# MatchaChoco010/toy-cpu-pathtracing

Hardware: NVIDIA B200
Metric: Mrays/s (higher is better)
Workload: dtype f32

## Files before the change

toy_cpu_pathtracing_b200/csrc/dcommon.cuh:

```cuda
#pragma once
#include <cuda_runtime.h>
#include <stdint.h>

#include "../../include/tcpt_flat.h"

namespace tcpt {

#define TCPT_PI 3.14159265358979323846f
#define TCPT_FLT_MAX 3.402823466e+38f
#define TCPT_INF __int_as_float(0x7f800000)

__device__ __forceinline__ float3 f3(float x, float y, float z) { return make_float3(x, y, z); }
__device__ __forceinline__ float3 operator+(float3 a, float3 b) { return f3(a.x + b.x, a.y + b.y, a.z + b.z); }
__device__ __forceinline__ float3 operator-(float3 a, float3 b) { return f3(a.x - b.x, a.y - b.y, a.z - b.z); }
__device__ __forceinline__ float3 operator-(float3 a) { return f3(-a.x, -a.y, -a.z); }
__device__ __forceinline__ float3 operator*(float3 a, float s) { return f3(a.x * s, a.y * s, a.z * s); }
__device__ __forceinline__ float3 operator*(float s, float3 a) { return f3(s * a.x, s * a.y, s * a.z); }
__device__ __forceinline__ float3 operator/(float3 a, float s) { return f3(a.x / s, a.y / s, a.z / s); }
__device__ __forceinline__ float dot(float3 a, float3 b) { return (a.x * b.x) + (a.y * b.y) + (a.z * b.z); }
__device__ __forceinline__ float3 cross(float3 a, float3 b) { return f3(a.y * b.z - b.y * a.z, a.z * b.x - b.z * a.x, a.x * b.y - b.x * a.y); }
__device__ __forceinline__ float length_squared(float3 a) { return dot(a, a); }
__device__ __forceinline__ float length(float3 a) { return sqrtf(dot(a, a)); }
__device__ __forceinline__ float3 normalize(float3 a) { return a * (1.0f / length(a)); }
__device__ __forceinline__ float comp(float3 a, int i) { return i == 0 ? a.x : (i == 1 ? a.y : a.z); }
// ... 11 lines not shown
    return f3((m[0] * v.x + m[3] * v.y) + m[6] * v.z, (m[1] * v.x + m[4] * v.y) + m[7] * v.z, (m[2] * v.x + m[5] * v.y) + m[8] * v.z);
}
__device__ __forceinline__ float3 xf_normal_by_inverse(const float* __restrict__ inv, float3 n) {
    float3 r = f3((inv[0] * n.x + inv[1] * n.y) + inv[2] * n.z, (inv[3] * n.x + inv[4] * n.y) + inv[5] * n.z, (inv[6] * n.x + inv[7] * n.y) + inv[8] * n.z);
    return normalize(r);
}

struct M3 { float3 c0, c1, c2; };
__device__ __forceinline__ M3 m3_inverse(const M3& s) {
    const float m00 = s.c0.x, m01 = s.c0.y, m02 = s.c0.z, m10 = s.c1.x, m11 = s.c1.y, m12 = s.c1.z, m20 = s.c2.x, m21 = s.c2.y, m22 = s.c2.z;
    M3 r;
    r.c0 = f3(m11 * m22 - m12 * m21, -(m01 * m22 - m02 * m21), m01 * m12 - m02 * m11);
    r.c1 = f3(-(m10 * m22 - m12 * m20), m00 * m22 - m02 * m20, -(m00 * m12 - m02 * m10));
    r.c2 = f3(m10 * m21 - m11 * m20, -(m00 * m21 - m01 * m20), m00 * m11 - m01 * m10);
    const float det = (m00 * r.c0.x + m01 * r.c1.x) + m02 * r.c2.x;
    const float rcp = 1.0f / det;
    r.c0 = r.c0 * rcp; r.c1 = r.c1 * rcp; r.c2 = r.c2 * rcp;
    return r;
}
__device__ __forceinline__ float3 m3_vector(const M3& m, float3 v) { return (m.c0 * v.x + m.c1 * v.y) + m.c2 * v.z; }
__device__ __forceinline__ float3 m3_normal_by_inverse(const M3& inv, float3 n) {
    return normalize(f3((inv.c0.x * n.x + inv.c0.y * n.y) + inv.c0.z * n.z, (inv.c1.x * n.x + inv.c1.y * n.y) + inv.c1.z * n.z,
                        (inv.c2.x * n.x + inv.c2.y * n.y) + inv.c2.z * n.z));
}

struct S4 { float v[4]; };
__device__ __forceinline__ S4 s4(float c) { S4 r; r.v[0] = r.v[1] = r.v[2] = r.v[3] = c; return r; }
__device__ __forceinline__ S4 s4(float4 a) { S4 r; r.v[0] = a.x; r.v[1] = a.y; r.v[2] = a.z; r.v[3] = a.w; return r; }
__device__ __forceinline__ float4 to_f4(const S4& a) { return make_float4(a.v[0], a.v[1], a.v[2], a.v[3]); }
#define S4_BINOP(op)                                                                                                   \
    __device__ __forceinline__ S4 operator op(const S4& a, const S4& b) { S4 r; _Pragma("unroll") for (int i = 0; i < 4; ++i) r.v[i] = a.v[i] op b.v[i]; return r; }
S4_BINOP(+) S4_BINOP(-) S4_BINOP(*)
__device__ __forceinline__ S4 operator*(const S4& a, float s) { S4 r; _Pragma("unroll") for (int i = 0; i < 4; ++i) r.v[i] = a.v[i] * s; return r; }
__device__ __forceinline__ S4 operator*(float s, const S4& a) { S4 r; _Pragma("unroll") for (int i = 0; i < 4; ++i) r.v[i] = s * a.v[i]; return r; }
__device__ __forceinline__ S4 operator/(const S4& a, float s) { S4 r; _Pragma("unroll") for (int i = 0; i < 4; ++i) r.v[i] = s == 0.0f ? 0.0f : a.v[i] / s; return r; }
__device__ __forceinline__ S4 operator/(const S4& a, const S4& b) { S4 r; _Pragma("unroll") for (int i = 0; i < 4; ++i) r.v[i] = b.v[i] == 0.0f ? 0.0f : a.v[i] / b.v[i]; return r; }
__device__ __forceinline__ float s4_max(const S4& a) { return rmax(rmax(rmax(rmax(-TCPT_INF, a.v[0]), a.v[1]), a.v[2]), a.v[3]); }
__device__ __forceinline__ float s4_avg(const S4& a) { return ((((0.0f + a.v[0]) + a.v[1]) + a.v[2]) + a.v[3]) / 4.0f; }
__device__ __forceinline__ bool s4_is_constant(const S4& a) { return a.v[1] == a.v[0] && a.v[2] == a.v[0] && a.v[3] == a.v[0]; }
__device__ __forceinline__ S4 s4_sqrt(const S4& a) { S4 r; _Pragma("unroll") for (int i = 0; i < 4; ++i) r.v[i] = sqrtf(a.v[i]); return r; }
__device__ __forceinline__ S4 s4_clamp(const S4& a, float lo, float hi) { S4 r; _Pragma("unroll") for (int i = 0; i < 4; ++i) r.v[i] = clampf(a.v[i], lo, hi); return r; }

struct DTexture { const uint8_t* data; uint32_t w, h, channels, pad; };
struct DEnv {
    const float* data; const float* marginal; const float* conditional;
    const uint32_t* marginal_guide; const uint32_t* conditional_guide; uint32_t guide_h, guide_w;
    float intensity, total_weight; uint32_t w, h; tcpt_flat_spectrum integrated; int32_t primitive;
    const float4* nee_table;
};
struct DScene {
    const float4* nodes;
    const int2* tlas_items;
    const float4* tri_verts;
    const float* positions; const float* normals; const float* uvs; const uint32_t* indices; const float* tangents;
    const tcpt_flat_geometry* geometries;
    const tcpt_flat_primitive* primitives; uint32_t n_primitives;
    const tcpt_flat_material* materials;
    const uint8_t* prim_mat_type;
    const DTexture* textures;
    const float* area_list; const float* area_table;
    int32_t light_list[TCPT_MAX_LIGHTS]; uint32_t n_lights;
    uint32_t one_light_always_on;
    const DEnv* envs; uint32_t n_envs;
    const float4* cmf;
    const float* z_nodes; const float* rgb2spec;
    float half_lin; int32_t half_zi;
    const float* presets;
    float xyz_to_rgb[9];
};

struct DCamera { float3 s, u, nf; float scale, aspect; };

struct DRender {
    uint32_t width, height, spp, seed, max_depth;
    int32_t integrator, sampler;
    float exposure;
    uint32_t log2_spp, n_base4_digits;
    uint32_t n_pix, pix_begin, s_begin, s_count, row_offset, row_stride;
    const uint32_t* pix_list;
    uint64_t n_pix_magic, width_magic;
    const uint32_t* sobol_prefix; uint32_t prefix_dims, prefix_stride;
    uint32_t pass_info;
    const unsigned long long* sobol_hash;
};
#define TCPT_SOBOL_HASH_N 512

typedef uint2 OrderEntry;

struct DState {
    float4* thr; float4* con; float4* fprev; float4* misc;
    float4* ppos;
    float4* rgb;
    float4* ext_o[2]; float4* ext_d[2];
    float4* hit0; uint2* hit1;
    float4* sh_o; float4* sh_d; float4* sh_c;
    OrderEntry* order; uint32_t capacity;
    uint32_t* counters;
    unsigned long long* stats;
};

enum : uint32_t { FLAG_SPEC_PREV = 1u, FLAG_LAMBDA_TERMINATED = 2u, FLAG_SAMPLED_PREV = 4u };

__constant__ uint32_t c_sobol_dim1[52];
__constant__ const uint32_t* c_sobol_dim1_bytes;

__device__ __forceinline__ uint32_t div_magic(uint32_t n, uint64_t magic) { return magic ? (uint32_t)__umul64hi((uint64_t)n, magic) : n; }
struct SobolFrame {
    const uint32_t* prefix;
    uint32_t prefix_stride, tables;
    uint32_t cfg;
    uint32_t seed;
    const unsigned long long* hash_table;
};
struct DSampler {
    uint32_t morton, dim, key, pix;

    __device__ __forceinline__ static uint32_t part1by1(uint32_t x) {
        x &= 0x0000ffffu;
        x = (x ^ (x << 8)) & 0x00ff00ffu;
        x = (x ^ (x << 4)) & 0x0f0f0f0fu;
        x = (x ^ (x << 2)) & 0x33333333u;
        x = (x ^ (x << 1)) & 0x55555555u;
        return x;
    }
    __device__ __forceinline__ static uint64_t mix_bits(uint64_t v) {
        v ^= v >> 31; v *= 0x7fb5d329728ea185ull; v ^= v >> 27; v *= 0x81dadef4bc2dd44dull; v ^= v >> 33;
        return v;
    }
    __device__ __forceinline__ static uint64_t hash(uint32_t dimension, uint32_t seed) {
        const uint64_t M = 0xc6a4a7935bd1e995ull;
        uint64_t h = 8ull * M;
        uint64_t k = (uint64_t)dimension | ((uint64_t)seed << 32);
        k *= M; k ^= k >> 47; k *= M;
        h ^= k; h *= M;
        h ^= h >> 47; h *= M; h ^= h >> 47;
        return h;
    }
    __device__ __forceinline__ static uint64_t hash_of(uint32_t k, const SobolFrame& f) {
        if (f.hash_table != nullptr && k < (uint32_t)TCPT_SOBOL_HASH_N) return __ldg(f.hash_table + k);
        return hash(k, f.seed);
    }
    __device__ __forceinline__ static uint32_t owen(uint32_t v, uint32_t seed) {
        v = __brev(v);
        v ^= v * 0x3d20adeau; v += seed; v *= (seed >> 16) | 1u; v ^= v * 0x05526c56u; v ^= v * 0x53a22864u;
        return __brev(v);
    }
    __device__ __forceinline__ static uint32_t pcg_hash2(uint32_t key, uint32_t ctr) {
        uint32_t x = key * 747796405u + ctr * 2891336453u + 0x9e3779b9u;
        x ^= x >> 16; x *= 0x7feb352du; x ^= x >> 15; x *= 0x846ca68bu; x ^= x >> 16;
        uint32_t w = ((x >> ((x >> 28u) + 4u)) ^ x) * 277803737u;
        return (w >> 22u) ^ w;
    }
    __device__ __forceinline__ static float unit_float(uint32_t x) { return (float)(x >> 8) * 5.9604644775390625e-8f; }
    __device__ __forceinline__ static float to_unit(uint32_t v) { return fminf((float)v * 2.3283064365386963e-10f, 0.99999994f); }

    __device__ __forceinline__ static uint32_t morton_of(uint32_t px, uint32_t py, uint32_t sample_index, uint32_t log2_spp) {
        return (((part1by1(py) << 1) | part1by1(px)) << log2_spp) | sample_index;
    }
    __device__ __forceinline__ void start(const DRender& R, uint32_t px, uint32_t py, uint32_t sample_index) {
        dim = 0;
        morton = morton_of(px, py, sample_index, R.log2_spp);
        key = (px * 0x9e3779b9u) ^ (py * 0x85ebca6bu) ^ (sample_index * 0xc2b2ae35u) ^ R.seed;
        pix = py * R.width + px;
    }
    __device__ __forceinline__ static SobolFrame frame_of(const DRender& R) {
        SobolFrame f;
// ... 344 lines not shown
```

toy_cpu_pathtracing_b200/csrc/kernels.cuh:

```cuda
#pragma once
#include "dshade.cuh"
#include "dtraverse.cuh"

#define TCPT_N_BUCKETS 9
#ifndef TCPT_SHADE_MIN_BLOCKS_LAMBERT
#define TCPT_SHADE_MIN_BLOCKS_LAMBERT 4
#endif
#ifndef TCPT_TRACE_MIN_BLOCKS
#define TCPT_TRACE_MIN_BLOCKS 8
#endif
#define TCPT_BUCKET_STRIDE 10

namespace tcpt {

struct PathList { const uint32_t* xy; const uint32_t* sample; };

__device__ __forceinline__ uint32_t owned_pixel(const DRender& R, uint32_t p_local) {
    return R.pix_list ? __ldg(R.pix_list + R.pix_begin + p_local) : R.pix_begin + p_local;
}

__device__ __forceinline__ void path_coords(const DRender& R, const PathList& L, uint32_t slot, uint32_t* px, uint32_t* py, uint32_t* si) {
    if (L.xy) { *px = __ldg(L.xy + 2 * (size_t)slot); *py = __ldg(L.xy + 2 * (size_t)slot + 1); *si = __ldg(L.sample + slot); return; }
    const uint32_t s_local = div_magic(slot, R.n_pix_magic), p_local = slot - s_local * R.n_pix;
    const uint32_t k = owned_pixel(R, p_local);
// ... 166 lines not shown
        const uint32_t b = bucket_of(sc, h.prim, killed);
        const uint32_t peers = __match_any_sync(__activemask(), b);
        const uint32_t lane = threadIdx.x & 31u;
        const int leader = __ffs(peers) - 1;
        uint32_t base = 0;
        if ((int)lane == leader) base = atomicAdd(&bcount[b], (uint32_t)__popc(peers));
        return CommitToken{base, peers, b, i, __float_as_uint(dw) & 0x7fffffffu};
    }
    __device__ __forceinline__ void end(const CommitToken& t) const {
        const uint32_t lane = threadIdx.x & 31u, peers = t.b, b = t.c, i = t.d;
        const uint32_t base = __shfl_sync(peers, t.a, __ffs(peers) - 1);
        st.order[(size_t)b * st.capacity + base + (uint32_t)__popc(peers & ((1u << lane) - 1u))] = make_uint2(i, t.e);
    }
};
struct CommitShadow {
    const DScene& sc; const DRender& R; const DState& st;
    __device__ __forceinline__ CommitToken begin(uint32_t i, const DHit& h) const {
        const uint32_t tag = __float_as_uint(st.sh_d[i].w);
        return CommitToken{tag, i, h.prim < 0 ? 1u : 0u, 0u, 0u};
    }
    __device__ __forceinline__ void end(const CommitToken& t) const {
        const uint32_t tag = t.a, i = t.b;
        const uint32_t slot = tag & 0x7fffffffu;
        const bool visible = t.c != 0u, last = (tag & 0x80000000u) != 0;
        if (!visible && !last) return;
        S4 con = s4(st.con[slot]);
        if (visible) {
            con = con + s4(st.sh_c[i]);
            st.con[slot] = to_f4(con);
        }
        if (last) {
            const float4 misc = st.misc[slot];
            const DWavelengths wl = wavelengths_uniform(misc.y, (__float_as_uint(misc.w) & FLAG_LAMBDA_TERMINATED) != 0);
            const float3 rgb = sensor_rgb(sc, wl.lambda[0], wl.terminated, con, R.exposure);
            st.rgb[slot] = make_float4(rgb.x, rgb.y, rgb.z, 0.0f);
        }
    }
};

template <bool COUNT>
__global__ void __launch_bounds__(128, 6) k_trace_closest(const __grid_constant__ DScene sc, const float4* __restrict__ q_o, const float4* __restrict__ q_d,
                                                        float4* __restrict__ hit0, uint2* __restrict__ hit1, const __grid_constant__ DState st, int cur) {
    const uint32_t n = st.counters[cur];
    uint32_t* bcount = st.counters + 4 + TCPT_BUCKET_STRIDE * cur;
    if (blockIdx.x == 0 && threadIdx.x == 0) {
        st.counters[cur ^ 1] = 0; st.counters[2] = 0; st.counters[25] = 0;
        for (int b = 0; b < TCPT_N_BUCKETS; ++b) st.counters[4 + TCPT_BUCKET_STRIDE * (cur ^ 1) + b] = 0;
        atomicAdd(&st.stats[0], (unsigned long long)n);
    }
    uint32_t nb = 0, nt = 0;
    __shared__ TraceShared ts;
    trace_queue<false, COUNT>(sc, ts, q_o, q_d, n, &st.counters[24], &nb, &nt, CommitClosest{sc, st, q_d, hit0, hit1, bcount});
    if (COUNT) { atomicAdd(&st.stats[2], (unsigned long long)nb); atomicAdd(&st.stats[3], (unsigned long long)nt); }
}

template <bool COUNT>
__global__ void __launch_bounds__(128, 6) k_trace_shadow(const __grid_constant__ DScene sc, const __grid_constant__ DRender R, const __grid_constant__ DState st) {
    const uint32_t n = st.counters[2];
    if (blockIdx.x == 0 && threadIdx.x == 0) atomicAdd(&st.stats[1], (unsigned long long)n);
    uint32_t nb = 0, nt = 0;
    __shared__ TraceShared ts;
    trace_queue<true, COUNT>(sc, ts, st.sh_o, st.sh_d, n, &st.counters[25], &nb, &nt, CommitShadow{sc, R, st});
    if (COUNT) { atomicAdd(&st.stats[2], (unsigned long long)nb); atomicAdd(&st.stats[3], (unsigned long long)nt); }
}

template <bool COUNT>
__global__ void __launch_bounds__(128, TCPT_TRACE_MIN_BLOCKS) k_trace_fused(const __grid_constant__ DScene sc, const __grid_constant__ DRender R, const __grid_constant__ DState st, int cur, int sh, uint32_t refill_lanes, uint32_t max_chunk) {
    const uint32_t n_sh = st.counters[sh], n = st.counters[cur];
    uint32_t* bcount = st.counters + 4 + TCPT_BUCKET_STRIDE * cur;
    if (blockIdx.x == 0 && threadIdx.x == 0) {
        st.counters[cur ^ 1] = 0; st.counters[sh ^ 1] = 0;
        for (int b = 0; b < TCPT_N_BUCKETS; ++b) st.counters[4 + TCPT_BUCKET_STRIDE * (cur ^ 1) + b] = 0;
        atomicAdd(&st.stats[0], (unsigned long long)n);
        atomicAdd(&st.stats[1], (unsigned long long)n_sh);
    }
    uint32_t nb = 0, nt = 0;
    __shared__ TraceShared ts;
    if (n_sh) trace_queue<true, COUNT>(sc, ts, st.sh_o, st.sh_d, n_sh, &st.counters[25], &nb, &nt, CommitShadow{sc, R, st}, refill_lanes, max_chunk);
    float4* __restrict__ hit0 = st.hit0; uint2* __restrict__ hit1 = st.hit1;
    if (n) trace_queue<false, COUNT>(sc, ts, st.ext_o[cur], st.ext_d[cur], n, &st.counters[24], &nb, &nt, CommitClosest{sc, st, st.ext_d[cur], hit0, hit1, bcount}, refill_lanes, max_chunk);
    if (COUNT) { atomicAdd(&st.stats[2], (unsigned long long)nb); atomicAdd(&st.stats[3], (unsigned long long)nt); }
}

struct ShadeOut {
    bool push_ext, push_sh;
    float4 eo, ed, so, sd, sc;
};

template <int B> struct BucketInfo {
    static constexpr bool miss = B == 7;
    static constexpr bool terminal = B == 8;
    static constexpr int mat = B == 0 ? TCPT_MAT_CLEARCOAT_PBR : B == 1 ? TCPT_MAT_SIMPLE_PBR : B == 2 ? TCPT_MAT_PLASTIC : B == 3 ? TCPT_MAT_GLASS : B == 4 ? TCPT_MAT_METAL
                              : B == 5 ? TCPT_MAT_LAMBERT : TCPT_MAT_EMISSIVE;
};

template <int B, bool FIRST = false>
__device__ __forceinline__ void shade_vertex(const DScene& sc, const DRender& R, const DState& st, const PathList& L, uint32_t stage_in,
                                             float3 ray_d, uint32_t slot, const float4 h0, const uint2 h1, const float4 misc, ShadeOut& out) {
    constexpr int MT = BucketInfo<B>::mat;
    const uint32_t stage = FIRST ? 0u : stage_in;
    out.push_ext = false; out.push_sh = false;
    float pdf_prev = misc.x;
    const float lambda0 = misc.y;
    uint32_t flags = __float_as_uint(misc.w);
    DWavelengths wl = wavelengths_uniform(lambda0, (flags & FLAG_LAMBDA_TERMINATED) != 0);
    uint32_t px, py, si;
    path_coords(R, L, slot, &px, &py, &si);
    DSampler smp = make_sampler(R, px, py, si);
    smp.dim = __float_as_uint(misc.z);
    constexpr bool NO_LOBE = MT == TCPT_MAT_LAMBERT || MT == TCPT_MAT_METAL;
    constexpr bool PRE = MT == TCPT_MAT_LAMBERT;
    DSampler::Draws3 pre; bool have_pre = false; const uint32_t pre_d0 = smp.dim;
    if (PRE && R.sampler == TCPT_SAMPLER_SOBOL && R.integrator != TCPT_INTEGRATOR_PT && (FIRST || stage < R.max_depth)) {
        pre = DSampler::sobol_draws3(smp.morton, pre_d0 + 1u, pre_d0 + 5u, pre_d0 + 7u, smp.pix, DSampler::frame_of(R));
        have_pre = true;
    }
    S4 thr = s4(1.0f), con = s4(0.0f);
    if (!FIRST && stage != 0u) { thr = s4(st.thr[slot]); con = s4(st.con[slot]); }
    const int integrator = R.integrator;
    constexpr bool miss = BucketInfo<B>::miss;

    auto finish = [&]() {
        const float3 rgb = sensor_rgb(sc, wl.lambda[0], wl.terminated, con, R.exposure);
        st.rgb[slot] = make_float4(rgb.x, rgb.y, rgb.z, 0.0f);
    };
    LightTable lt; bool lt_ready = false;
    auto lights = [&]() -> const LightTable& {
        if (!lt_ready) {
            if (sc.one_light_always_on) { lt.w[0] = 1.0f; lt.sum = 1.0f; }
            else light_table(sc, wl, lt);
            lt_ready = true;
        }
        return lt;
    };

    if constexpr (BucketInfo<B>::terminal) {
        const S4 zero = s4(0.0f);
        const bool spec_prev = (flags & FLAG_SPEC_PREV) != 0;
        if (integrator == TCPT_INTEGRATOR_PT) con = con + thr * zero;
        else if (integrator == TCPT_INTEGRATOR_NEE || spec_prev) { if (spec_prev) con = con + thr * zero; }
        else {
            const float a = pdf_prev, b = 0.0f;
            const float w = (a == 0.0f && b == 0.0f) ? 0.0f : a / (a + b);
            con = con + thr * zero * w;
        }
        finish();
        return;
    }
    if constexpr (miss) {
        if (sc.n_envs != 0) {
            if (FIRST || stage == 0) {
                S4 radiance;
                scene_env_radiance_pdf(sc, nullptr, ray_d, wl, &radiance, nullptr);
                con = con + thr * radiance;
            } else if (integrator != TCPT_INTEGRATOR_NEE) {
                const S4 fprev = s4(st.fprev[slot]);
                if (integrator == TCPT_INTEGRATOR_PT) {
                    S4 radiance;
                    scene_env_radiance_pdf(sc, nullptr, ray_d, wl, &radiance, nullptr);
                    con = con + thr * fprev * radiance / pdf_prev;
                } else {
                    S4 radiance; float light_pdf;
                    scene_env_radiance_pdf(sc, &lights(), ray_d, wl, &radiance, &light_pdf);
                    const float a = pdf_prev, b = light_pdf;
                    const float w = (a == 0.0f && b == 0.0f) ? 0.0f : a / (a + b);
                    const float tf = 1.0f / pdf_prev;
                    con = con + thr * fprev * radiance * tf * w;
                }
            }
        }
        finish();
        return;
    } else {

    DSurface hit;
    reconstruct_hit(sc, (int)h1.x, h1.y, h0.y, h0.z, h0.w, ray_d, hit);
    const tcpt_flat_material& mat = sc.materials[hit.material];
    constexpr bool emissive = MT == TCPT_MAT_EMISSIVE;

    if (FIRST || stage == 0) {
        if (emissive) con = con + thr * emissive_radiance(sc, mat, hit.uv, wl);
    } else {
        const S4 fprev = s4(st.fprev[slot]);
        const float tf = 1.0f / pdf_prev;
        S4 next_emissive = s4(0.0f);
        if (emissive) next_emissive = fprev * emissive_radiance(sc, mat, hit.uv, wl) * tf;
        const S4 modifier = fprev * tf;
        const bool spec_prev = (flags & FLAG_SPEC_PREV) != 0;
        if (integrator == TCPT_INTEGRATOR_PT) {
            con = con + thr * next_emissive;
        } else if (integrator == TCPT_INTEGRATOR_NEE) {
            if (spec_prev) con = con + thr * next_emissive;
        } else {
            if (spec_prev) con = con + thr * next_emissive;
            else {
                const float4 pp = st.ppos[slot];
                const float pdf_light = scene_pdf_light_sample(sc, lights(), f3(pp.x, pp.y, pp.z), hit.prim, hit.tri, hit.position, hit.normal);
                const float a = pdf_prev, b = pdf_light;
                const float w = (a == 0.0f && b == 0.0f) ? 0.0f : a / (a + b);
                con = con + thr * next_emissive * w;
            }
        }
        thr = thr * modifier;
        const float p_rr = s4_max(thr);
        if (!emissive && !(p_rr >= 1.0f) && p_rr != 0.0f) { thr.v[0] /= p_rr; thr.v[1] /= p_rr; thr.v[2] /= p_rr; thr.v[3] /= p_rr; }
    }
    if (stage >= R.max_depth || emissive) { finish(); return; }
    if constexpr (!emissive) {

    M3 r2t, t2r;
    shading_frame(hit, r2t, t2r);
    const float3 wo = m3_vector(r2t, hit.wo);
    const float3 ng_t = m3_normal_by_inverse(t2r, hit.normal);
    MatCtx mc; mc.sc = &sc; mc.path_key = smp.key; mc.depth = stage + 1;
    float uc = 0.0f;
    if (NO_LOBE) smp.skip_1d();
    else uc = smp.get_1d(R);
    float2 uv;
    if (PRE && have_pre && smp.dim == pre_d0 + 1u) { uv = pre.a; smp.dim += 2; } else uv = smp.get_2d(R);
    const bool was_terminated = wl.terminated;
    NmFrame nmf;
    material_frame(sc, mat, hit.uv, nmf);
    MatParams mp;
    load_mat_params<MT>(sc, mat, hit.uv, wl, mp);
    mc.mp = &mp;
    const MatSample ms = material_sample<MT>(mc, mat, nmf, uc, uv, wl, wo, ng_t, hit.uv);
    if (wl.terminated != was_terminated) lt_ready = false;

    if (!ms.is_specular() && integrator != TCPT_INTEGRATOR_PT) {
        const bool with_mis = integrator == TCPT_INTEGRATOR_MIS;
        float p_light = 0.0f;
        int li;
        if (sc.n_lights == 1) {
            smp.skip_1d();
            const LightTable& t1 = lights();
            li = t1.sum == 0.0f ? -1 : 0;
            p_light = t1.w[0] / t1.sum;
        } else {
            const float u = smp.get_1d(R);
            li = sample_light(sc, lights(), u, &p_light);
        }
        if (li >= 0) {
            const int lprim = sc.light_list[li];
            const tcpt_flat_primitive& LP = sc.primitives[lprim];
            float s = 0.0f;
            if (LP.kind == 1) s = smp.get_1d(R); else smp.skip_1d();
            float2 luv = make_float2(0.0f, 0.0f);
            if (LP.kind <= 2) { if (PRE && have_pre && smp.dim == pre_d0 + 5u) { luv = pre.b; smp.dim += 2; } else luv = smp.get_2d(R); }
            else { smp.skip_1d(); smp.skip_1d(); }
            float3 sh_dir; float sh_tmax; S4 pending; float sh_eps = 1e-4f;
            if (LP.kind == 3 || LP.kind == 4) {
                const float3 lpos = xf_point(LP.l2r, f3(0.0f, 0.0f, 0.0f));
                S4 inten = spectrum_sample(sc, spectrum_from_flat(LP.light_spectrum), wl) * LP.light_intensity;
                const float3 dv = lpos - hit.position;
                const float3 wi_r = normalize(dv);
                if (LP.kind == 4) {
                    const float cos_theta = xf_vector(LP.r2l, wi_r).z;
                    const float t = clampf((cos_theta - LP.angle_outer) / (LP.angle_inner - LP.angle_outer), 0.0f, 1.0f);
                    inten = inten * (t * t * (3.0f - 2.0f * t));
                }
                const float3 wi = m3_vector(r2t, wi_r);
                S4 f; float bpdf;
                material_eval_pdf<MT>(mc, mat, nmf, wl, wo, wi, ng_t, hit.uv, false, &f, &bpdf);
                pending = thr * (f * inten / (length_squared(dv) * p_light));
                sh_dir = wi_r; sh_tmax = length(dv) - 2.0f * 1e-4f;
            } else if (LP.kind == 5) {
                const float3 dir = normalize(xf_vector(LP.l2r, f3(0.0f, 0.0f, 1.0f)));
                const S4 inten = spectrum_sample(sc, spectrum_from_flat(LP.light_spectrum), wl) * LP.light_intensity;
                const float3 wi = m3_vector(r2t, normalize(dir));
                S4 f; float bpdf;
                material_eval_pdf<MT>(mc, mat, nmf, wl, wo, wi, ng_t, hit.uv, false, &f, &bpdf);
                pending = thr * (f * inten / p_light);
                sh_dir = dir; sh_tmax = TCPT_FLT_MAX; sh_eps = 0.0f;
            } else if (LP.kind == 2) {
                const DEnv& e = sc.envs[LP.env];
                const uint32_t yy = sample_from_cdf(e.marginal, e.h, e.marginal_guide, e.guide_h, luv.x);
                const uint32_t xx = sample_from_cdf(e.conditional + (size_t)yy * e.w, e.w, e.conditional_guide + (size_t)yy * (e.guide_w + 1u), e.guide_w, luv.y);
                const EnvNee en = env_nee_lookup(sc, LP, e, xx, yy);
                const float3 wi_r = en.wi_r;
                const float pdf_dir = en.pdf_dir;
                const S4 radiance = spectrum_sample(sc, en.spec, wl) * e.intensity;
                const float3 wi = m3_vector(r2t, wi_r);
                S4 f; float bpdf;
                material_eval_pdf<MT>(mc, mat, nmf, wl, wo, wi, ng_t, hit.uv, with_mis, &f, &bpdf);
                const float w = with_mis ? ((pdf_dir == 0.0f && bpdf == 0.0f) ? 0.0f : pdf_dir / (pdf_dir + bpdf)) : 1.0f;
                const S4 c = f * radiance / (pdf_dir * p_light);
                pending = with_mis ? thr * c * w : thr * c;
                sh_dir = wi_r; sh_tmax = TCPT_FLT_MAX;
            } else {
                const tcpt_flat_geometry& G = sc.geometries[LP.geometry];
                const float* table = sc.area_table + LP.area_base;
                uint32_t index = 0;
                for (uint32_t i = 0; i < G.tri_count; ++i) if (s < __ldg(table + i)) { index = i; break; }
                float b0, b1;
                if (luv.x < luv.y) { b0 = luv.x / 2.0f; b1 = luv.y - b0; } else { b1 = luv.y / 2.0f; b0 = luv.x - b1; }
                const float b2 = 1.0f - b0 - b1;
                const uint32_t* idx = sc.indices + 3 * ((size_t)G.index_base + index);
                const uint32_t i0 = __ldg(idx) + G.vertex_base, i1 = __ldg(idx + 1) + G.vertex_base, i2 = __ldg(idx + 2) + G.vertex_base;
                const float* pp = sc.positions;
                const float3 p0 = xf_point(LP.l2r, f3(__ldg(pp + 3 * (size_t)i0), __ldg(pp + 3 * (size_t)i0 + 1), __ldg(pp + 3 * (size_t)i0 + 2)));
                const float3 p1 = xf_point(LP.l2r, f3(__ldg(pp + 3 * (size_t)i1), __ldg(pp + 3 * (size_t)i1 + 1), __ldg(pp + 3 * (size_t)i1 + 2)));
                const float3 p2 = xf_point(LP.l2r, f3(__ldg(pp + 3 * (size_t)i2), __ldg(pp + 3 * (size_t)i2 + 1), __ldg(pp + 3 * (size_t)i2 + 2)));
                const float3 lpos = (p0 * b0 + p1 * b1) + p2 * b2;
                const float3 lnormal = normalize(normalize(cross(p1 - p0, p2 - p0)));
                float2 tuv = make_float2(0.0f, 0.0f);
                if (G.has_uv) {
                    const float* uu = sc.uvs;
                    tuv.x = (__ldg(uu + 2 * (size_t)i0) * b0 + __ldg(uu + 2 * (size_t)i1) * b1) + __ldg(uu + 2 * (size_t)i2) * b2;
                    tuv.y = (__ldg(uu + 2 * (size_t)i0 + 1) * b0 + __ldg(uu + 2 * (size_t)i1 + 1) * b1) + __ldg(uu + 2 * (size_t)i2 + 1) * b2;
                }
                if (G.single) tuv = luv;
                const float3 dv = lpos - hit.position;
                const float3 wi_r = normalize(dv);
                const S4 radiance = emissive_radiance(sc, sc.materials[LP.material], tuv, wl);
                const float pdf_area = 1.0f / LP.area_sum;
                const float distance = length(dv);
                const float pdf_dir = pdf_area * (distance * distance) / rmax(fabsf(dot(lnormal, -wi_r)), 1e-8f);
                const float3 wi = m3_vector(r2t, wi_r);
                S4 f; float bpdf;
                material_eval_pdf<MT>(mc, mat, nmf, wl, wo, wi, ng_t, hit.uv, with_mis, &f, &bpdf);
                const float distance2 = length_squared(dv);
                const float3 ln_t = m3_normal_by_inverse(t2r, lnormal);
                const float cos_light = fabsf(dot(ln_t, -wi));
                const float g = cos_light / distance2;
                const float w = with_mis ? ((pdf_dir == 0.0f && bpdf == 0.0f) ? 0.0f : pdf_dir / (pdf_dir + bpdf)) : 1.0f;
                const S4 c = f * radiance * g / (pdf_area * p_light);
                pending = with_mis ? thr * c * w : thr * c;
                sh_dir = wi_r; sh_tmax = distance - 2.0f * 1e-4f;
            }
            const float3 so = sh_eps != 0.0f ? hit.position + sh_dir * sh_eps : hit.position;
            out.push_sh = true;
            out.so = make_float4(so.x, so.y, so.z, sh_tmax);
            out.sd = make_float4(sh_dir.x, sh_dir.y, sh_dir.z, __uint_as_float(slot));
            out.sc = to_f4(pending);
        }
    }

    if (!ms.sampled) {
        st.con[slot] = to_f4(con);
        if (out.push_sh) {
            out.sd.w = __uint_as_float(slot | 0x80000000u);
            st.misc[slot] = make_float4(0.0f, lambda0, __uint_as_float(smp.dim), __uint_as_float(wl.terminated ? FLAG_LAMBDA_TERMINATED : 0u));
        } else finish();
        return;
    }
    const float3 wi_render = m3_vector(t2r, ms.wi);
    const float sign = dot(hit.normal, wi_render) < 0.0f ? -1.0f : 1.0f;
    const float3 origin = hit.position + (sign * hit.normal) * 1e-5f;
    const float3 o2 = origin + wi_render * 1e-5f;
    bool killed = false;
    if (stage + 1 <= R.max_depth) {
        const S4 thr2 = thr * (ms.f * (1.0f / ms.pdf));
        const float p_rr = s4_max(thr2);
        if (!(p_rr >= 1.0f)) {
            float u_rr;
            if (PRE && have_pre && smp.dim == pre_d0 + 7u) { u_rr = pre.c; smp.dim += 1; } else u_rr = smp.get_1d(R);
            killed = !(u_rr < p_rr);
        }
    }
    out.push_ext = true;
    out.eo = make_float4(o2.x, o2.y, o2.z, TCPT_FLT_MAX);
    out.ed = make_float4(wi_render.x, wi_render.y, wi_render.z, __uint_as_float(slot | (killed ? 0x80000000u : 0u)));
    st.thr[slot] = to_f4(thr);
    st.con[slot] = to_f4(con);
    st.fprev[slot] = to_f4(ms.f);
    st.ppos[slot] = make_float4(hit.position.x, hit.position.y, hit.position.z, 0.0f);
    flags = (ms.is_specular() ? FLAG_SPEC_PREV : 0u) | (wl.terminated ? FLAG_LAMBDA_TERMINATED : 0u);
    st.misc[slot] = make_float4(ms.pdf, lambda0, __uint_as_float(smp.dim), __uint_as_float(flags));
    }
    }
}

struct VertexIn { float4 d, h0, misc; uint2 h1; };
template <int B>
__device__ __forceinline__ OrderEntry load_order(const DState& st, uint32_t p, uint32_t n) {
    OrderEntry o = make_uint2(0u, 0u);
    if (p < n) o = st.order[(size_t)B * st.capacity + p];
    return o;
}
template <int B>
__device__ __forceinline__ VertexIn load_vertex(const DState& st, int cur, OrderEntry o, bool valid) {
    VertexIn v;
    v.d = make_float4(0.0f, 0.0f, 0.0f, 0.0f); v.h0 = v.d; v.misc = v.d; v.h1 = make_uint2(0u, 0u);
    if (valid) {
        const uint32_t i = o.x;
        v.misc = st.misc[o.y];
        v.d = st.ext_d[cur][i];
        if (B < 7) { v.h0 = st.hit0[i]; v.h1 = st.hit1[i]; }
    }
    return v;
}
__device__ __forceinline__ void push_rays(const DState& st, int cur, int sh, int b, const ShadeOut& out) {
    if (b < 6) {
        uint32_t pe, ps;
        warp_push2(&st.counters[cur ^ 1], out.push_ext, &st.counters[sh], out.push_sh, &pe, &ps);
        if (out.push_ext) { st.ext_o[cur ^ 1][pe] = out.eo; st.ext_d[cur ^ 1][pe] = out.ed; }
        if (out.push_sh) { st.sh_o[ps] = out.so; st.sh_d[ps] = out.sd; st.sh_c[ps] = out.sc; }
    }
}

#ifndef TCPT_SHADE_THREADS
#define TCPT_SHADE_THREADS 512
#endif
#ifndef TCPT_SHADE_THREADS_LAMBERT
#define TCPT_SHADE_THREADS_LAMBERT TCPT_SHADE_THREADS
#endif
#ifndef TCPT_SHADE_THREADS_MISS
#define TCPT_SHADE_THREADS_MISS TCPT_SHADE_THREADS
#endif
#ifndef TCPT_SHADE_MIN_BLOCKS_MISS
#define TCPT_SHADE_MIN_BLOCKS_MISS 8
#endif
template <int B> struct ShadeCfg {
    static constexpr int threads = B >= 6 ? TCPT_SHADE_THREADS_MISS : B == 5 ? TCPT_SHADE_THREADS_LAMBERT : TCPT_SHADE_THREADS;
    static constexpr int per_sm_128 = B >= 6 ? TCPT_SHADE_MIN_BLOCKS_MISS : B == 5 ? TCPT_SHADE_MIN_BLOCKS_LAMBERT : TCPT_SHADE_MIN_BLOCKS;
    static constexpr int min_blocks = per_sm_128 * 128 / threads > 0 ? per_sm_128 * 128 / threads : 1;
};
template <int B, bool FIRST = false>
__global__ void __launch_bounds__(ShadeCfg<B>::threads, ShadeCfg<B>::min_blocks) k_shade(const __grid_constant__ DScene sc, const __grid_constant__ DRender R,
                                                                                     const __grid_constant__ DState st, const __grid_constant__ PathList L, int cur, int sh, uint32_t stage) {
    if (B == 0 && blockIdx.x == 0 && threadIdx.x == 0) { st.counters[24] = 0; st.counters[25] = 0; }
    const uint32_t stride = gridDim.x * blockDim.x;
    const uint32_t n = st.counters[4 + TCPT_BUCKET_STRIDE * cur + B];
    const uint32_t unit = B < 6 ? (uint32_t)ShadeCfg<B>::threads : 32u;
    const uint32_t n_round = (n + unit - 1u) / unit * unit;
    uint32_t p = blockIdx.x * blockDim.x + threadIdx.x;
    VertexIn v = load_vertex<B>(st, cur, load_order<B>(st, p, n), p < n);
    for (; p < n_round; p += stride) {
        const uint32_t pn = p + stride;
        const bool more = pn < n && pn > p;
        const OrderEntry o_next = load_order<B>(st, pn, more ? n : 0u);
        if (B < 6) __syncthreads();
        ShadeOut out; out.push_ext = false; out.push_sh = false;
        if (p < n) shade_vertex<B, FIRST>(sc, R, st, L, stage, f3(v.d.x, v.d.y, v.d.z), __float_as_uint(v.d.w) & 0x7fffffffu, v.h0, v.h1, v.misc, out);
        push_rays(st, cur, sh, B, out);
        v = load_vertex<B>(st, cur, o_next, more);
    }
}

// ... 282 lines not shown
```

toy_cpu_pathtracing_b200/csrc/tcpt_api.cu:

```cuda
#include <cuda_runtime.h>
#include <dlfcn.h>
#include "host_image.h"
#include "host_obj.h"
#include <nccl.h>

#include <algorithm>
#include <cmath>
#include <cstdio>
#include <cstring>
#include <mutex>
#include <string>
#include <thread>
#include <vector>

#include "../../include/tcpt.h"
#include "../../include/tcpt_flat.h"
#include "host_scene.h"
#include "kernels.cuh"
#include "lbvh.cuh"

using namespace tcpt;

namespace {

// ... 231 lines not shown
        const size_t need = n_pix * (dims + 2 * pass_rows);
        if (need > ctx->prefix_cap) {
            if (ctx->d_prefix) { cudaStreamSynchronize(stream); cudaFree(ctx->d_prefix); ctx->d_prefix = nullptr; ctx->prefix_cap = 0; }
            if (cudaMalloc((void**)&ctx->d_prefix, need * 4) != cudaSuccess) { cudaGetLastError(); ctx->prefix_dims = 0; return TCPT_OK; }
            ctx->prefix_cap = need;
        }
        cudaEvent_t a, b; cudaEventCreate(&a); cudaEventCreate(&b);
        cudaEventRecord(a, stream);
        const size_t total = n_pix * dims;
        const int grid = (int)((total + 255) / 256 < (size_t)ctx->sm_count * 64 ? (total + 255) / 256 : (size_t)ctx->sm_count * 64);
        k_sobol_prefix<<<grid, 256, 0, stream>>>(ctx->d_prefix, R.width, R.height, R.log2_spp, R.n_base4_digits, (uint32_t)dims);
        cudaEventRecord(b, stream);
        CU(cudaEventSynchronize(b));
        float ms = 0.0f; cudaEventElapsedTime(&ms, a, b); ctx->prefix_build_ms = ms; ctx->stats.sobol_prefix_ms = ms;
        cudaEventDestroy(a); cudaEventDestroy(b);
        CU(cudaGetLastError());
        if (pass_rows) CU(cudaMemsetAsync(ctx->d_prefix + n_pix * (dims + pass_rows), 0, n_pix * pass_rows * 4, stream));
        ctx->prefix_w = R.width; ctx->prefix_h = R.height; ctx->prefix_log2spp = R.log2_spp; ctx->prefix_dims = (uint32_t)dims; ctx->pass_rows = (uint32_t)pass_rows;
    }
    R.sobol_prefix = ctx->d_prefix; R.prefix_dims = ctx->prefix_dims; R.prefix_stride = (uint32_t)n_pix;
    ctx->stats.sobol_prefix_bytes = (uint64_t)n_pix * ctx->prefix_dims * 4;
    return TCPT_OK;
}

struct StageTimer {
    tcpt_ctx* ctx; bool on; int stage; size_t slot;
    StageTimer(tcpt_ctx* c, int stage_id, cudaStream_t s) : ctx(c), on(c->opt.stage_timing != 0), stage(stage_id), slot(0) {
        if (!on) return;
        slot = ctx->ev_used;
        while (ctx->ev_pool.size() < slot + 2) { cudaEvent_t e; cudaEventCreate(&e); ctx->ev_pool.push_back(e); }
        ctx->ev_used += 2;
        ctx->ev_stage.push_back(stage);
        cudaEventRecord(ctx->ev_pool[slot], s);
        stream = s;
    }
    ~StageTimer() { if (on) cudaEventRecord(ctx->ev_pool[slot + 1], stream); }
    cudaStream_t stream = nullptr;
};
enum { STAGE_GENERATE = 0, STAGE_CLOSEST = 1, STAGE_SHADE = 2, STAGE_SHADOW = 3, STAGE_FILM = 4 };

void build_sobol_pass(tcpt_ctx* ctx, DRender& Rp, cudaStream_t stream) {
    Rp.pass_info = 0;
    if (!Rp.sobol_prefix || ctx->pass_rows == 0 || (Rp.log2_spp & 1u) || Rp.log2_spp > 16u || Rp.s_count < 4u) return;
    uint32_t v = 0;
    while ((Rp.s_begin >> v) != ((Rp.s_begin + Rp.s_count - 1u) >> v)) ++v;
    const uint32_t iv = (v + 1u) >> 1;
    const size_t total = (size_t)Rp.n_pix * ctx->pass_rows;
    const int grid = (int)((total + 255) / 256 < (size_t)ctx->sm_count * 64 ? (total + 255) / 256 : (size_t)ctx->sm_count * 64);
    StageTimer t(ctx, STAGE_GENERATE, stream);
    const uint32_t half = Rp.log2_spp >> 1;
    if (ctx->opt.sobol_pass_cache && iv >= 1u && iv <= 7u && half >= iv + 1u && half - iv <= 4u)
        k_sobol_pass_cached<<<grid_for(ctx, Rp.n_pix, 256), 256, 0, stream>>>(ctx->d_prefix, Rp, ctx->pass_rows, iv, ctx->prefix_dims + ctx->pass_rows);
    else
        k_sobol_pass<<<grid, 256, 0, stream>>>(ctx->d_prefix, Rp, ctx->pass_rows, iv);
    ctx->stats.kernel_launches++;
    Rp.pass_info = ctx->pass_rows | (iv << 8);
}

void collect_stage_times(tcpt_ctx* ctx) {
    double* acc[5] = {&ctx->stats.generate_ms, &ctx->stats.trace_closest_ms, &ctx->stats.shade_ms, &ctx->stats.trace_shadow_ms, &ctx->stats.film_ms};
    for (size_t i = 0; i < ctx->ev_stage.size(); ++i) {
        float ms = 0.0f;
        if (cudaEventElapsedTime(&ms, ctx->ev_pool[2 * i], ctx->ev_pool[2 * i + 1]) == cudaSuccess) *acc[ctx->ev_stage[i]] += ms;
    }
    ctx->ev_used = 0;
    ctx->ev_stage.clear();
}

static void debug_dump(tcpt_ctx* ctx, const char* what, uint32_t stage, int cur, cudaStream_t stream) {
    const DState& st = ctx->st;
    cudaStreamSynchronize(stream);
    uint32_t cnt[4]; float4 o, d, h0, thr, con, misc, so, sd, sc_; uint2 h1;
    cudaMemcpy(cnt, st.counters, sizeof cnt, cudaMemcpyDeviceToHost);
    cudaMemcpy(&o, st.ext_o[cur], 16, cudaMemcpyDeviceToHost); cudaMemcpy(&d, st.ext_d[cur], 16, cudaMemcpyDeviceToHost);
    cudaMemcpy(&h0, st.hit0, 16, cudaMemcpyDeviceToHost); cudaMemcpy(&h1, st.hit1, 8, cudaMemcpyDeviceToHost);
    cudaMemcpy(&thr, st.thr, 16, cudaMemcpyDeviceToHost); cudaMemcpy(&con, st.con, 16, cudaMemcpyDeviceToHost); cudaMemcpy(&misc, st.misc, 16, cudaMemcpyDeviceToHost);
    cudaMemcpy(&so, st.sh_o, 16, cudaMemcpyDeviceToHost); cudaMemcpy(&sd, st.sh_d, 16, cudaMemcpyDeviceToHost); cudaMemcpy(&sc_, st.sh_c, 16, cudaMemcpyDeviceToHost);
    uint32_t dim, fl; std::memcpy(&dim, &misc.z, 4); std::memcpy(&fl, &misc.w, 4);
    std::fprintf(stderr, "[tcpt %s stage %u] q=%u/%u sh=%u ray o(%.9g %.9g %.9g) d(%.9g %.9g %.9g) tmax %.9g | hit t %.9g prim %d tri %d | thr %.9g %.9g %.9g %.9g con %.9g %.9g %.9g %.9g pdf_prev %.9g dim %u flags %u | shadow o(%.9g %.9g %.9g) d(%.9g %.9g %.9g) tmax %.9g c %.9g %.9g %.9g %.9g\n",
                 what, stage, cnt[0], cnt[1], cnt[2], o.x, o.y, o.z, d.x, d.y, d.z, o.w, h0.x, (int)h1.x, (int)h1.y, thr.x, thr.y, thr.z, thr.w, con.x, con.y, con.z, con.w, misc.x, dim, fl,
                 so.x, so.y, so.z, sd.x, sd.y, sd.z, so.w, sc_.x, sc_.y, sc_.z, sc_.w);
}

int run_pass(tcpt_ctx* ctx, const DRender& R, const DCamera& cam, const PathList& L, uint32_t n_slots, float* dev_acc, cudaStream_t stream, float2* dev_mom = nullptr) {
    const DScene& sc = ctx->dev.view;
    const DState& st = ctx->st;
    const bool count = ctx->opt.count_tests != 0;
    {
        StageTimer t(ctx, STAGE_GENERATE, stream);
        if (ctx->opt.generate_pixels && L.xy == nullptr && R.sampler == TCPT_SAMPLER_SOBOL && R.s_count >= 2u && (uint64_t)R.n_pix * R.s_count == n_slots)
            k_generate_pixels<<<grid_for(ctx, R.n_pix, 256), 256, 0, stream>>>(sc, R, cam, st, n_slots);
        else
            k_generate<<<grid_for(ctx, n_slots, 256), 256, 0, stream>>>(sc, R, cam, st, L, n_slots);
        ctx->stats.kernel_launches++;
    }
    const int g128 = grid_for(ctx, n_slots, 128);
    auto shade_grid = [&](int threads) { return (int)std::max<uint64_t>(1, std::min<uint64_t>(((uint64_t)n_slots + threads - 1) / threads, (uint64_t)ctx->sm_count * ctx->opt.blocks_per_sm * 128 / threads)); };
#define TCPT_SHADE_LAUNCH(...) k_shade<__VA_ARGS__><<<shade_grid(ShadeCfg<TCPT_FIRST_ARG(__VA_ARGS__)>::threads), ShadeCfg<TCPT_FIRST_ARG(__VA_ARGS__)>::threads, 0, stream>>>(sc, R, st, L, cur, sh, stage)
#define TCPT_FIRST_ARG(a, ...) a
    if (R.integrator >= TCPT_INTEGRATOR_ALBEDO) {
        if (count) k_trace_fused<true><<<g128, 128, 0, stream>>>(sc, R, st, 0, 3, (uint32_t)ctx->opt.refill_b0, (uint32_t)ctx->opt.chunk_b0);
        else k_trace_fused<false><<<g128, 128, 0, stream>>>(sc, R, st, 0, 3, (uint32_t)ctx->opt.refill_b0, (uint32_t)ctx->opt.chunk_b0);
        k_aov<<<g128, 128, 0, stream>>>(sc, R, st);
        ctx->stats.kernel_launches += 2; ctx->stats.trace_launches++; ctx->stats.shade_launches++;
    } else {
    const bool fuse_trace = (ctx->opt.fused_launches & 1) != 0;
    for (uint32_t stage = 0; stage <= R.max_depth; ++stage) {
        const int cur = (int)(stage & 1u);
        const bool fuse_shade = (ctx->opt.fused_launches & 2) != 0 && stage >= (uint32_t)ctx->opt.fused_shade_from;
        const int sh = fuse_trace ? 2 + cur : 2, sh_prev = 2 + (int)((stage + 1u) & 1u);
        {
            StageTimer t(ctx, STAGE_CLOSEST, stream);
            if (fuse_trace) {
                if (count) k_trace_fused<true><<<g128, 128, 0, stream>>>(sc, R, st, cur, sh_prev, (uint32_t)(stage == 0 ? ctx->opt.refill_b0 : ctx->opt.refill), (uint32_t)(stage == 0 ? ctx->opt.chunk_b0 : ctx->opt.chunk));
                else k_trace_fused<false><<<g128, 128, 0, stream>>>(sc, R, st, cur, sh_prev, (uint32_t)(stage == 0 ? ctx->opt.refill_b0 : ctx->opt.refill), (uint32_t)(stage == 0 ? ctx->opt.chunk_b0 : ctx->opt.chunk));
            } else {
                if (count) k_trace_closest<true><<<g128, 128, 0, stream>>>(sc, st.ext_o[cur], st.ext_d[cur], st.hit0, st.hit1, st, cur);
                else k_trace_closest<false><<<g128, 128, 0, stream>>>(sc, st.ext_o[cur], st.ext_d[cur], st.hit0, st.hit1, st, cur);
            }
            ctx->stats.kernel_launches++; ctx->stats.trace_launches++;
        }
        {
            StageTimer t(ctx, STAGE_SHADE, stream);
            if (fuse_shade) {
                k_shade_all<<<g128, 128, 0, stream>>>(sc, R, st, L, cur, sh, stage);
                ctx->stats.kernel_launches++; ctx->stats.shade_launches++;
            } else {
                if (stage == 0) {
                    TCPT_SHADE_LAUNCH(0, true);
                    TCPT_SHADE_LAUNCH(1, true);
                    TCPT_SHADE_LAUNCH(2, true);
                    TCPT_SHADE_LAUNCH(3, true);
                    TCPT_SHADE_LAUNCH(4, true);
                    TCPT_SHADE_LAUNCH(5, true);
                    TCPT_SHADE_LAUNCH(6, true);
                    TCPT_SHADE_LAUNCH(7, true);
                    TCPT_SHADE_LAUNCH(8, true);
                } else {
                    TCPT_SHADE_LAUNCH(0);
                    TCPT_SHADE_LAUNCH(1);
                    TCPT_SHADE_LAUNCH(2);
                    TCPT_SHADE_LAUNCH(3);
                    TCPT_SHADE_LAUNCH(4);
                    TCPT_SHADE_LAUNCH(5);
                    TCPT_SHADE_LAUNCH(6);
                    TCPT_SHADE_LAUNCH(7);
                    TCPT_SHADE_LAUNCH(8);
                }
                ctx->stats.kernel_launches += 9; ctx->stats.shade_launches += 9;
            }
        }
        if (ctx->opt.debug_path_log && n_slots == 1) debug_dump(ctx, "after shade", stage, cur ^ 1, stream);
        if (!fuse_trace && R.integrator != TCPT_INTEGRATOR_PT && stage < R.max_depth) {
            StageTimer t(ctx, STAGE_SHADOW, stream);
            if (count) k_trace_shadow<true><<<g128, 128, 0, stream>>>(sc, R, st);
            else k_trace_shadow<false><<<g128, 128, 0, stream>>>(sc, R, st);
            ctx->stats.kernel_launches++; ctx->stats.trace_launches++;
        }
    }
    }
    if (dev_acc) {
        StageTimer t(ctx, STAGE_FILM, stream);
        if (dev_mom) k_film_moments<<<grid_for(ctx, R.n_pix, 256), 256, 0, stream>>>(R, st.rgb, dev_acc, dev_mom);
        else k_film<<<grid_for(ctx, R.n_pix, 256), 256, 0, stream>>>(R, st.rgb, dev_acc);
        ctx->stats.kernel_launches++;
    }
    ctx->stats.passes++;
    CU(cudaGetLastError());
    return TCPT_OK;
}

int fetch_stats(tcpt_ctx* ctx) {
    unsigned long long h[8];
    CU(cudaMemcpy(h, ctx->d_stats, sizeof h, cudaMemcpyDeviceToHost));
    ctx->stats.closest_rays = h[0]; ctx->stats.shadow_rays = h[1]; ctx->stats.box_tests = h[2]; ctx->stats.tri_tests = h[3]; ctx->stats.paths = h[4];
    return TCPT_OK;
}

void reset_stats(tcpt_ctx* ctx) {
    cudaMemsetAsync(ctx->d_stats, 0, 8 * sizeof(unsigned long long), ctx->stream);
    ctx->stats = tcpt_stats{};
    ctx->stats.max_bvh_depth = ctx->dev.max_bvh_depth;
    ctx->ev_used = 0; ctx->ev_stage.clear();
}

int render_passes(tcpt_ctx* ctx, const DRender& R, const DCamera& cam, uint64_t owned, const uint32_t* pix_list, uint32_t s0, uint32_t s1,
                  uint32_t max_slots, float* dev_acc, float2* dev_mom, cudaStream_t stream) {
    if (pix_list && dev_acc && !dev_mom) return fail(ctx, TCPT_ERR_INVALID, "render: a pass over a pixel list films through k_film_moments");
    int rc = TCPT_OK;
    uint64_t budget = max_slots;
    if (budget == 0) {
        if (ctx->default_slots == 0) {
            size_t free_b = 0, total_b = 0;
            if (cudaMemGetInfo(&free_b, &total_b) != cudaSuccess) { cudaGetLastError(); free_b = (size_t)16 << 30; }
            const uint64_t avail = (uint64_t)free_b + (uint64_t)ctx->st_capacity * kBytesPerSlot;
            uint64_t b = (uint64_t)(0.45 * (double)avail) / kBytesPerSlot;
            if (b > (128ull << 20)) b = 128ull << 20;
            if (b < (1ull << 20)) b = 1ull << 20;
            ctx->default_slots = b;
        }
        budget = ctx->default_slots;
    }
    if (budget > 0xffffffffull) budget = 0xffffffffull;
// ... 1136 lines not shown
```

Baseline: 4300.

## Precompute bounce-0 Sobol draws and env texel per pixel in a separate kernel

Adds a per-pixel kernel, run after the first closest-hit trace, that computes the bounce-0 Sobol samples (material lobe, direction, light select, light uv, Russian roulette) for all of a pixel's samples. It reuses per-pixel sample-index loads and presolves the environment CDF lookup to a texel. Shading at stage 0 reads these values from the thr/con/fprev buffers instead of evaluating the sampler and CDF search itself. The aim is to amortise per-pixel Sobol setup and take divergent CDF searches out of the shade kernels. The cost is an extra launch and extra global memory traffic to write and read the staged values.

```diff
diff --git a/toy_cpu_pathtracing_b200/csrc/dcommon.cuh b/toy_cpu_pathtracing_b200/csrc/dcommon.cuh
--- a/toy_cpu_pathtracing_b200/csrc/dcommon.cuh
+++ b/toy_cpu_pathtracing_b200/csrc/dcommon.cuh
@@ -117,6 +117,7 @@
     const uint32_t* sobol_prefix; uint32_t prefix_dims, prefix_stride;
     uint32_t pass_info;
     const unsigned long long* sobol_hash;
+    uint32_t b0_draws;
 };
 #define TCPT_SOBOL_HASH_N 512
 
diff --git a/toy_cpu_pathtracing_b200/csrc/kernels.cuh b/toy_cpu_pathtracing_b200/csrc/kernels.cuh
--- a/toy_cpu_pathtracing_b200/csrc/kernels.cuh
+++ b/toy_cpu_pathtracing_b200/csrc/kernels.cuh
@@ -272,6 +272,69 @@
     if (COUNT) { atomicAdd(&st.stats[2], (unsigned long long)nb); atomicAdd(&st.stats[3], (unsigned long long)nt); }
 }
 
+#define TCPT_B0_NO_TEXEL 0xffffffffu
+__global__ void __launch_bounds__(256) k_bounce0_draws(const __grid_constant__ DScene sc, const __grid_constant__ DRender R, const __grid_constant__ DState st) {
+    const uint32_t stride = gridDim.x * blockDim.x;
+    const SobolFrame f = DSampler::frame_of(R);
+    const uint64_t h4 = DSampler::hash_of(6u, f), h8 = DSampler::hash_of(10u, f);
+    const uint32_t h3 = (uint32_t)DSampler::hash_of(4u, f), h6 = (uint32_t)DSampler::hash_of(7u, f), h7 = (uint32_t)DSampler::hash_of(8u, f), h10 = (uint32_t)DSampler::hash_of(11u, f);
+    const bool one_env = sc.n_envs == 1 && sc.envs[0].w < 0xffffu && sc.envs[0].h < 0xffffu;
+    for (uint32_t p = blockIdx.x * blockDim.x + threadIdx.x; p < R.n_pix; p += stride) {
+        const uint32_t k = owned_pixel(R, p);
+        const uint32_t row = div_magic(k, R.width_magic);
+        const uint32_t px = k - row * R.width, py = R.row_offset + row * R.row_stride;
+        const uint32_t pix = py * R.width + px;
+        const uint32_t pixel_morton = DSampler::morton_of(px, py, 0u, R.log2_spp);
+        const DSampler::SobolLoads l3 = DSampler::sample_index_loads(3u, pix, f), l4 = DSampler::sample_index_loads(4u, pix, f), l6 = DSampler::sample_index_loads(6u, pix, f),
+                                   l7 = DSampler::sample_index_loads(7u, pix, f), l8 = DSampler::sample_index_loads(8u, pix, f), l10 = DSampler::sample_index_loads(10u, pix, f);
+        for (uint32_t s = 0; s < R.s_count; ++s) {
+            const uint32_t slot = s * R.n_pix + p;
+            if (bucket_of(sc, (int)st.hit1[slot].x, false) >= 6u) continue;
+            const uint32_t morton = pixel_morton | (R.s_begin + s);
+            const uint64_t a4 = DSampler::sample_index_from(morton, 4u, f, l4), a8 = DSampler::sample_index_from(morton, 8u, f, l8);
+            const float u3 = DSampler::to_unit(DSampler::owen(__brev((uint32_t)DSampler::sample_index_from(morton, 3u, f, l3)), h3));
+            const float u4 = DSampler::to_unit(DSampler::owen(__brev((uint32_t)a4), (uint32_t)h4)), u5 = DSampler::to_unit(DSampler::owen(DSampler::sobol_dim1(a4), (uint32_t)(h4 >> 32)));
+            const float u6 = DSampler::to_unit(DSampler::owen(__brev((uint32_t)DSampler::sample_index_from(morton, 6u, f, l6)), h6));
+            const float u7 = DSampler::to_unit(DSampler::owen(__brev((uint32_t)DSampler::sample_index_from(morton, 7u, f, l7)), h7));
+            const float u8 = DSampler::to_unit(DSampler::owen(__brev((uint32_t)a8), (uint32_t)h8)), u9 = DSampler::to_unit(DSampler::owen(DSampler::sobol_dim1(a8), (uint32_t)(h8 >> 32)));
+            const float u10 = DSampler::to_unit(DSampler::owen(__brev((uint32_t)DSampler::sample_index_from(morton, 10u, f, l10)), h10));
+            uint32_t texel = TCPT_B0_NO_TEXEL;
+            if (one_env) {
+                const DEnv& e = sc.envs[0];
+                const uint32_t yy = sample_from_cdf(e.marginal, e.h, e.marginal_guide, e.guide_h, u8);
+                const uint32_t xx = sample_from_cdf(e.conditional + (size_t)yy * e.w, e.w, e.conditional_guide + (size_t)yy * (e.guide_w + 1u), e.guide_w, u9);
+                texel = yy << 16 | xx;
+            }
+            st.thr[slot] = make_float4(u3, u4, u5, u6);
+            st.con[slot] = make_float4(u7, u8, u9, u10);
+            st.fprev[slot] = make_float4(__uint_as_float(texel), 0.0f, 0.0f, 0.0f);
+        }
+    }
+}
+
+template <bool EAGER>
+struct B0Draws {
+    const DRender& R; const DState& st; const uint32_t slot; const bool on;
+    float2 dir, luv; float rr; uint32_t texel;
+    __device__ __forceinline__ B0Draws(const DRender& R_, const DState& st_, uint32_t slot_, bool first) : R(R_), st(st_), slot(slot_), on(first && R_.b0_draws != 0u) {
+        if (EAGER && on) { dir = make_float2(a(1), a(2)); luv = make_float2(b(1), b(2)); rr = b(3); texel = __float_as_uint(st.fprev[slot].x); }
+    }
+    __device__ __forceinline__ float a(int i) const { return ((const float*)(st.thr + slot))[i]; }
+    __device__ __forceinline__ float b(int i) const { return ((const float*)(st.con + slot))[i]; }
+    __device__ __forceinline__ float get_1d(DSampler& smp) const {
+        const uint32_t d = smp.dim;
+        if (on && (d == 3u || d == 6u || d == 7u || d == 10u)) { smp.dim += 1; return d == 3u ? a(0) : d == 6u ? a(3) : d == 7u ? b(0) : EAGER ? rr : b(3); }
+        return smp.get_1d(R);
+    }
+    __device__ __forceinline__ float2 get_2d(DSampler& smp) const {
+        const uint32_t d = smp.dim;
+        if (on && d == 4u) { smp.dim += 2; return EAGER ? dir : make_float2(a(1), a(2)); }
+        if (on && d == 8u) { smp.dim += 2; return EAGER ? luv : make_float2(b(1), b(2)); }
+        return smp.get_2d(R);
+    }
+    __device__ __forceinline__ uint32_t env_texel() const { return EAGER ? texel : __float_as_uint(st.fprev[slot].x); }
+};
+
 struct ShadeOut {
     bool push_ext, push_sh;
     float4 eo, ed, so, sd, sc;
@@ -299,9 +362,10 @@
     DSampler smp = make_sampler(R, px, py, si);
     smp.dim = __float_as_uint(misc.z);
     constexpr bool NO_LOBE = MT == TCPT_MAT_LAMBERT || MT == TCPT_MAT_METAL;
-    constexpr bool PRE = MT == TCPT_MAT_LAMBERT;
+    constexpr bool PRE = MT == TCPT_MAT_LAMBERT && !FIRST;
+    const B0Draws<MT == TCPT_MAT_LAMBERT> b0(R, st, slot, FIRST);
     DSampler::Draws3 pre; bool have_pre = false; const uint32_t pre_d0 = smp.dim;
-    if (PRE && R.sampler == TCPT_SAMPLER_SOBOL && R.integrator != TCPT_INTEGRATOR_PT && (FIRST || stage < R.max_depth)) {
+    if (PRE && R.sampler == TCPT_SAMPLER_SOBOL && R.integrator != TCPT_INTEGRATOR_PT && stage < R.max_depth) {
         pre = DSampler::sobol_draws3(smp.morton, pre_d0 + 1u, pre_d0 + 5u, pre_d0 + 7u, smp.pix, DSampler::frame_of(R));
         have_pre = true;
     }
@@ -405,9 +469,9 @@
     MatCtx mc; mc.sc = &sc; mc.path_key = smp.key; mc.depth = stage + 1;
     float uc = 0.0f;
     if (NO_LOBE) smp.skip_1d();
-    else uc = smp.get_1d(R);
+    else uc = b0.get_1d(smp);
     float2 uv;
-    if (PRE && have_pre && smp.dim == pre_d0 + 1u) { uv = pre.a; smp.dim += 2; } else uv = smp.get_2d(R);
+    if (PRE && have_pre && smp.dim == pre_d0 + 1u) { uv = pre.a; smp.dim += 2; } else uv = b0.get_2d(smp);
     const bool was_terminated = wl.terminated;
     NmFrame nmf;
     material_frame(sc, mat, hit.uv, nmf);
@@ -427,16 +491,17 @@
             li = t1.sum == 0.0f ? -1 : 0;
             p_light = t1.w[0] / t1.sum;
         } else {
-            const float u = smp.get_1d(R);
+            const float u = b0.get_1d(smp);
             li = sample_light(sc, lights(), u, &p_light);
         }
         if (li >= 0) {
             const int lprim = sc.light_list[li];
             const tcpt_flat_primitive& LP = sc.primitives[lprim];
             float s = 0.0f;
-            if (LP.kind == 1) s = smp.get_1d(R); else smp.skip_1d();
+            if (LP.kind == 1) s = b0.get_1d(smp); else smp.skip_1d();
             float2 luv = make_float2(0.0f, 0.0f);
-            if (LP.kind <= 2) { if (PRE && have_pre && smp.dim == pre_d0 + 5u) { luv = pre.b; smp.dim += 2; } else luv = smp.get_2d(R); }
+            const bool luv_ahead = b0.on && smp.dim == 8u;
+            if (LP.kind <= 2) { if (PRE && have_pre && smp.dim == pre_d0 + 5u) { luv = pre.b; smp.dim += 2; } else luv = b0.get_2d(smp); }
             else { smp.skip_1d(); smp.skip_1d(); }
             float3 sh_dir; float sh_tmax; S4 pending; float sh_eps = 1e-4f;
             if (LP.kind == 3 || LP.kind == 4) {
@@ -464,8 +529,13 @@
                 sh_dir = dir; sh_tmax = TCPT_FLT_MAX; sh_eps = 0.0f;
             } else if (LP.kind == 2) {
                 const DEnv& e = sc.envs[LP.env];
-                const uint32_t yy = sample_from_cdf(e.marginal, e.h, e.marginal_guide, e.guide_h, luv.x);
-                const uint32_t xx = sample_from_cdf(e.conditional + (size_t)yy * e.w, e.w, e.conditional_guide + (size_t)yy * (e.guide_w + 1u), e.guide_w, luv.y);
+                uint32_t yy, xx;
+                const uint32_t texel = luv_ahead ? b0.env_texel() : TCPT_B0_NO_TEXEL;
+                if (texel != TCPT_B0_NO_TEXEL) { yy = texel >> 16; xx = texel & 0xffffu; }
+                else {
+                    yy = sample_from_cdf(e.marginal, e.h, e.marginal_guide, e.guide_h, luv.x);
+                    xx = sample_from_cdf(e.conditional + (size_t)yy * e.w, e.w, e.conditional_guide + (size_t)yy * (e.guide_w + 1u), e.guide_w, luv.y);
+                }
                 const EnvNee en = env_nee_lookup(sc, LP, e, xx, yy);
                 const float3 wi_r = en.wi_r;
                 const float pdf_dir = en.pdf_dir;
@@ -544,7 +614,7 @@
         const float p_rr = s4_max(thr2);
         if (!(p_rr >= 1.0f)) {
             float u_rr;
-            if (PRE && have_pre && smp.dim == pre_d0 + 7u) { u_rr = pre.c; smp.dim += 1; } else u_rr = smp.get_1d(R);
+            if (PRE && have_pre && smp.dim == pre_d0 + 7u) { u_rr = pre.c; smp.dim += 1; } else u_rr = b0.get_1d(smp);
             killed = !(u_rr < p_rr);
         }
     }
diff --git a/toy_cpu_pathtracing_b200/csrc/tcpt_api.cu b/toy_cpu_pathtracing_b200/csrc/tcpt_api.cu
--- a/toy_cpu_pathtracing_b200/csrc/tcpt_api.cu
+++ b/toy_cpu_pathtracing_b200/csrc/tcpt_api.cu
@@ -337,13 +337,16 @@
                  so.x, so.y, so.z, sd.x, sd.y, sd.z, so.w, sc_.x, sc_.y, sc_.z, sc_.w);
 }
 
-int run_pass(tcpt_ctx* ctx, const DRender& R, const DCamera& cam, const PathList& L, uint32_t n_slots, float* dev_acc, cudaStream_t stream, float2* dev_mom = nullptr) {
+int run_pass(tcpt_ctx* ctx, const DRender& R_pass, const DCamera& cam, const PathList& L, uint32_t n_slots, float* dev_acc, cudaStream_t stream, float2* dev_mom = nullptr) {
     const DScene& sc = ctx->dev.view;
     const DState& st = ctx->st;
     const bool count = ctx->opt.count_tests != 0;
+    const bool per_pixel = ctx->opt.generate_pixels && L.xy == nullptr && R_pass.sampler == TCPT_SAMPLER_SOBOL && R_pass.s_count >= 2u && (uint64_t)R_pass.n_pix * R_pass.s_count == n_slots;
+    DRender R = R_pass;
+    R.b0_draws = per_pixel && R.integrator < TCPT_INTEGRATOR_ALBEDO && R.max_depth >= 1u && !((ctx->opt.fused_launches & 2) != 0 && ctx->opt.fused_shade_from <= 0) ? 1u : 0u;
     {
         StageTimer t(ctx, STAGE_GENERATE, stream);
-        if (ctx->opt.generate_pixels && L.xy == nullptr && R.sampler == TCPT_SAMPLER_SOBOL && R.s_count >= 2u && (uint64_t)R.n_pix * R.s_count == n_slots)
+        if (per_pixel)
             k_generate_pixels<<<grid_for(ctx, R.n_pix, 256), 256, 0, stream>>>(sc, R, cam, st, n_slots);
         else
             k_generate<<<grid_for(ctx, n_slots, 256), 256, 0, stream>>>(sc, R, cam, st, L, n_slots);
@@ -374,6 +377,11 @@
                 else k_trace_closest<false><<<g128, 128, 0, stream>>>(sc, st.ext_o[cur], st.ext_d[cur], st.hit0, st.hit1, st, cur);
             }
             ctx->stats.kernel_launches++; ctx->stats.trace_launches++;
+        }
+        if (stage == 0 && R.b0_draws) {
+            StageTimer t(ctx, STAGE_GENERATE, stream);
+            k_bounce0_draws<<<grid_for(ctx, R.n_pix, 256), 256, 0, stream>>>(sc, R, st);
+            ctx->stats.kernel_launches++;
         }
         {
             StageTimer t(ctx, STAGE_SHADE, stream);
```

Result: faster. 4387 (median of 6 runs) (+2.0%).
